# Yash-10/beta-sgp

Measured on AMD Instinct MI355X. Metric: SGP iterations/sec (fp64) on batched 256x256 images, higher is better.
Workload: dtype f64; 1 GPU; C3: 1024 independent 256x256 stamps per GPU, 25x25 PSF, linear A, beta-SGP (beta=1.05), proj_type=1, MAXIT=100, stop_criterion=1; images_per_gpu=1024, images_total=1024, maxit=100, parallelism=1 independent shards, one process per GPU (no collective on the data path), ls_spec=2, streams=1, team=1, proj_cache=1, gn_compact=1, storage=f64, persistent=1, stop_criterion=1

## Files before the change

beta-sgp_amd/csrc/bsgp_device.hpp:

```cpp
#pragma once

#include <hip/hip_runtime.h>
#include <stdint.h>

#include <type_traits>

#include "bsgp_fft.hpp"
#include "bsgp_math.hpp"

namespace bsgp {

#ifndef BSGP_BLOCK
#define BSGP_BLOCK 256
#endif
constexpr int kBlock = BSGP_BLOCK;
constexpr int kWaves = kBlock / 64;
constexpr int kMaxRed = 24;

constexpr int kTeamFlags = 64;
constexpr int kPartBufs = 3;
constexpr unsigned long long kPartEmpty = 0xFFF75EE0FFF75EE0ull;
constexpr unsigned int kPartEmptyWord = 0xFFF75EE0u;
constexpr int kSharedBytes = 512;

constexpr int kPhaseSlots = 32;
#ifdef BSGP_PHASE_PROF
static __device__ unsigned long long g_phase[kPhaseSlots];
#define PH_T(v) const unsigned long long v = __builtin_amdgcn_s_memtime()
#define PH_ADD(slot, t0)                                                                 \
  do {                                                                                   \
    if (threadIdx.x == 0) atomicAdd(&g_phase[slot], __builtin_amdgcn_s_memtime() - (t0)); \
  } while (0)
#define PH_SUB(slot, t)                                                                 \
  do {                                                                                  \
    if (PHS >= 0) {                                                                     \
      const unsigned long long t_ = __builtin_amdgcn_s_memtime();                        \
      if (threadIdx.x == 0) atomicAdd(&g_phase[(slot) < 0 ? 0 : (slot)], t_ - (t));       \
      t = t_;                                                                           \
    }                                                                                   \
  } while (0)
#define PH_SUB_T(v) unsigned long long v = __builtin_amdgcn_s_memtime()
#else
#define PH_T(v)
#define PH_ADD(slot, t0)
#define PH_SUB(slot, t)
#define PH_SUB_T(v)
#endif

struct Geo {
  int H, W;
  int P, Q;
  int Qh;
  int nfw;
  int nfc;
  int coop;
  int lpad;
  int sld;
  int tw2;
  int twmix;
  FftPlan fp;
  FftPlan fq;
  const cd* tfA;
  const cd* tfAT;
  size_t tf_stride;
};

__device__ __forceinline__ const cd* tf_of(const Geo& G, int img, int transpose) {
  return (transpose ? G.tfAT : G.tfA) + (size_t)img * G.tf_stride;
}

__device__ __forceinline__ void copy_tw(const FftPlan& f) {
  if (f.lds_tw < 0) return;
  extern __shared__ __attribute__((aligned(16))) char bsgp_dyn_lds[];
  cd* d = reinterpret_cast<cd*>(bsgp_dyn_lds + f.lds_tw);
  for (int i = threadIdx.x; i < f.n; i += kBlock) d[i] = f.tw[i];
}
__device__ __forceinline__ void copy_tw2(const FftPlan& f) {
  if (f.lds_tw2 < 0) return;
  extern __shared__ __attribute__((aligned(16))) char bsgp_dyn_lds[];
  cd* d = reinterpret_cast<cd*>(bsgp_dyn_lds + f.lds_tw2);
  const int m = 64 + f.n / 64;
  for (int i = threadIdx.x; i < m; i += blockDim.x) d[i] = f.tw[i < 64 ? i : 64 * (i - 64)];
}
__device__ __forceinline__ void load_tw_lds(const Geo& G) {
  if (G.twmix >= 0) {
    extern __shared__ __attribute__((aligned(16))) char bsgp_dyn_lds[];
    cd* d = reinterpret_cast<cd*>(bsgp_dyn_lds + G.twmix);
    for (int i = threadIdx.x; i < 64 + 512; i += blockDim.x)
      d[i] = G.fp.tw[i < 64 ? 32 * i : 4 * (i - 64)];
  }
// ... 558 lines not shown
    if (v != v) v = __longlong_as_double(0x7ff8000000000000ll);
    st_sc1(slot + (size_t)t.m * kMaxRed, v);
  }
  team_red_barrier(t);
  if (threadIdx.x < 64) {
    const int lane = threadIdx.x;
    double s;
    unsigned int spins = 0;
    for (;;) {
      bool ok = true;
      s = MAX ? -INFINITY : INFINITY;
      for (int mm = lane; mm < t.T; mm += 64) {
        const double u = ld_sc1(slot + (size_t)mm * kMaxRed);
        ok &= !part_empty(u);
        s = MAX ? ((u > s || u != u) ? u : s) : ((u < s || u != u) ? u : s);
      }
      if (red_poll_done(t, ok, spins)) break;
    }
    s = MAX ? wave_max(s) : wave_min(s);
    if (lane == 0) red[kWaves * kMaxRed] = s;
  }
  __syncthreads();
  const double r = red[kWaves * kMaxRed];
  __syncthreads();
  team_red_done(t);
  return r;
}
__device__ __forceinline__ double team_max(double v, double* red, Team& t) {
  return team_ext<true>(v, red, t);
}
__device__ __forceinline__ double team_min(double v, double* red, Team& t) {
  return team_ext<false>(v, red, t);
}

__device__ __forceinline__ double fpow(double x, double a) {
#ifdef BSGP_VALU_X2
  const double x2 = x + 0.0 * a * x;
  const double r1 = exp(a * fast_log(x));
  const double r2 = exp(a * fast_log(x2));
  return r1 == r2 ? r1 : r2;
#else
  return exp(a * fast_log(x));
#endif
}

__device__ __forceinline__ double np_max2(double a, double b) {
  return (a != a || b != b) ? (a + b) : (a > b ? a : b);
}
__device__ __forceinline__ double np_min2(double a, double b) {
  return (a != a || b != b) ? (a + b) : (a < b ? a : b);
}
__device__ __forceinline__ double py_max2(double a, double b) { return (b > a) ? b : a; }
__device__ __forceinline__ double py_min2(double a, double b) { return (b < a) ? b : a; }

struct alignas(32) CPair {
  cd a, b;
};

__device__ __forceinline__ void store_pair(cd* col, bool two, bool pair_ok, cd ak, cd bk) {
  if (two && pair_ok) {
    CPair v;
    v.a = ak;
    v.b = bk;
    *reinterpret_cast<CPair*>(col) = v;
  } else {
    col[0] = ak;
    if (two) col[1] = bk;
  }
}

constexpr int kJCH = 4;
constexpr int kGCH = 3;
constexpr int kPCH = 5;

template <int JCH, class LD, class V>
__device__ __forceinline__ void load_rows(LD& ld, int r, bool two, int j0, int lane, int ncols,
                                          V (&v0)[JCH], V (&v1)[JCH]) {
  const int r1 = two ? r + 1 : r;
#pragma unroll
  for (int u = 0; u < JCH; ++u) {
    const int j = min(j0 + lane + 64 * u, ncols - 1);
    v0[u] = ld(r, j);
    v1[u] = ld(r1, j);
  }
}

struct BlockSync {
  __device__ __forceinline__ void operator()() const { __syncthreads(); }
};
constexpr int kCCH = 4;


template <class LD, class MK>
__device__ __forceinline__ void coop_row_fwd_1(const Geo& G, const Part& D, int nrows, int ncols,
                                             int ldim, cd* spec, cd* lds, LD& ld, MK& mk) {
  using V = decltype(ld(0, 0));
  const int t = threadIdx.x;
  const bool pair_ok = (ldim & 1) == 0;
  cd* a = lds;
  cd* b = lds + G.lpad;
  for (int r = 2 * D.gw0; r < nrows; r += 2 * D.gws) {
    const bool two = (r + 1) < nrows;
    for (int j0 = 0; j0 < G.Q; j0 += kBlock * kCCH) {
      V v0[kCCH], v1[kCCH];
#pragma unroll
      for (int u = 0; u < kCCH; ++u) {
        const int j = min(j0 + t + kBlock * u, ncols - 1);
        v0[u] = ld(r, j);
        v1[u] = ld(two ? r + 1 : r, j);
      }
#pragma unroll
      for (int u = 0; u < kCCH; ++u) {
        const int j = j0 + t + kBlock * u;
        if (j < G.Q) {
          double va = 0.0, vb = 0.0;
          if (j < ncols) {
            va = mk(r, j, v0[u]);
            if (two) vb = mk(r + 1, j, v1[u]);
          }
          a[j] = cmk(va, vb);
        }
      }
    }
    __syncthreads();
    cd* Z = fft_wide(a, b, G.fq, false, t, kBlock, BlockSync());
    for (int k = t; k < G.Qh; k += kBlock) {
      cd ak, bk;
      r2c_split(Z, G.Q, k, &ak, &bk);
      store_pair(spec + (size_t)k * ldim + r, two, pair_ok, ak, bk);
    }
    __syncthreads();
  }
}

__device__ __forceinline__ void coop_gather_1(const Geo& G, const cd* spec, int r, bool two, cd* a) {
  const int t = threadIdx.x;
  for (int k0 = 0; k0 < G.Qh; k0 += kBlock * kCCH) {
    cd A[kCCH], B[kCCH];
#pragma unroll
    for (int u = 0; u < kCCH; ++u) {
      const int k = min(k0 + t + kBlock * u, G.Qh - 1);
      const cd* col = spec + (size_t)k * G.sld + r;
      A[u] = col[0];
      const cd b = col[two ? 1 : 0];
      B[u] = two ? b : cmk(0.0, 0.0);
    }
#pragma unroll
    for (int u = 0; u < kCCH; ++u) {
      const int k = k0 + t + kBlock * u;
      if (k < G.Qh) {
        a[k] = cmk(A[u].x - B[u].y, A[u].y + B[u].x);
        if (k > 0 && G.Q - k >= G.Qh) a[G.Q - k] = cmk(A[u].x + B[u].y, B[u].x - A[u].y);
      }
    }
  }
  __syncthreads();
}

template <class LD, class USE>
__device__ __forceinline__ void coop_row_inv_1(const Geo& G, const Part& D, const cd* spec, cd* lds,
                                             LD& ld, USE& use) {
  using V = decltype(ld(0, 0));
  const int t = threadIdx.x;
  cd* a = lds;
  cd* b = lds + G.lpad;
  for (int r = 2 * D.gw0; r < G.H; r += 2 * D.gws) {
// ... 331 lines not shown
  const int t = c.t;
  cd* a = lds + c.g * 2 * G.lpad;
  cd* b = a + G.lpad;
  for (int k0 = D.gw0; k0 < G.Qh; k0 += D.gws) {
    const int k = k0 + c.g;
    const bool act = k < G.Qh;
    cd* col = spec + (size_t)k * G.sld;
    const cd* tk = tf + (size_t)k * G.P;
    PH_T(tq0);
    if (act) {
      for (int p0 = 0; p0 < G.P; p0 += c.nt * kCCH) {
        cd cv[kCCH];
#pragma unroll
        for (int u = 0; u < kCCH; ++u) {
          const int p = p0 + t + c.nt * u;
          const cd v = col[min(p, G.H - 1)];
          cv[u] = (p < G.H) ? v : cmk(0.0, 0.0);
        }
#pragma unroll
        for (int u = 0; u < kCCH; ++u) {
          const int p = p0 + t + c.nt * u;
          if (p < G.P) a[p] = cv[u];
        }
      }
    }
    __syncthreads();
    PH_ADD(29, tq0);
    PH_T(tq1);
    cd* Z = fft_wide<false>(a, b, G.fp, false, t, c.nt, BlockSync());
    if (act) {
      for (int p0 = 0; p0 < G.P; p0 += c.nt * kCCH) {
        cd tv[kCCH];
#pragma unroll
        for (int u = 0; u < kCCH; ++u) tv[u] = tk[min(p0 + t + c.nt * u, G.P - 1)];
#pragma unroll
        for (int u = 0; u < kCCH; ++u) {
          const int p = p0 + t + c.nt * u;
          if (p < G.P) Z[p] = cmul(Z[p], tv[u]);
        }
      }
    }
    __syncthreads();
    cd* Y = fft_wide<false>(Z, (Z == a) ? b : a, G.fp, true, t, c.nt, BlockSync());
    if (act)
      for (int p = t; p < G.H; p += c.nt) col[p] = Y[p];
    __syncthreads();
    PH_ADD(30, tq1);
  }
}

template <class LD, class MK>
__device__ __forceinline__ void coop_row_fwd(const Geo& G, const Part& D, int nrows, int ncols,
                                             int ldim, cd* spec, cd* lds, LD& ld, MK& mk) {
  if (D.nf == 1)
    coop_row_fwd_1(G, D, nrows, ncols, ldim, spec, lds, ld, mk);
  else
    coop_row_fwd_g(G, D, nrows, ncols, ldim, spec, lds, ld, mk);
}
template <class LD, class USE>
__device__ __forceinline__ void coop_row_inv(const Geo& G, const Part& D, const cd* spec, cd* lds,
                                             LD& ld, USE& use) {
  if (D.nf == 1)
    coop_row_inv_1(G, D, spec, lds, ld, use);
  else
    coop_row_inv_g(G, D, spec, lds, ld, use);
}
template <class CP>
__device__ __forceinline__ void coop_row_inv_fwd(const Geo& G, const Part& D, cd* spec, cd* lds,
                                                 CP& cp) {
  if (D.nf == 1)
    coop_row_inv_fwd_1(G, D, spec, lds, cp);
  else
    coop_row_inv_fwd_g(G, D, spec, lds, cp);
}
__device__ __forceinline__ void coop_col_conv(const Geo& G, const Part& D, cd* spec, const cd* tf,
                                              cd* lds) {
  if (D.nf == 1)
    coop_col_conv_1(G, D, spec, tf, lds);
  else
    coop_col_conv_g(G, D, spec, tf, lds);
}

template <int JCH = kJCH, bool PF = false, bool COMP = true, bool COOP = false,
          bool PIPE = false, int PHS = -1, class LD, class MK>
__device__ __forceinline__ void row_fwd2(const Geo& G, const Part& D, int nrows, int ncols,
                                         int ldim, cd* spec, cd* lds, LD&& ld, MK&& mk) {
  if constexpr (COOP) {
    coop_row_fwd(G, D, nrows, ncols, ldim, spec, lds, ld, mk);
    return;
  }
  using V = decltype(ld(0, 0));
  const int w = threadIdx.x >> 6, lane = threadIdx.x & 63;
  const bool pair_ok = (ldim & 1) == 0;
  if (w < G.nfw) {
    cd* a = lds + w * 2 * G.lpad;
    cd* b = a + G.lpad;
    int r = 2 * (D.gw0 + w);
    V v0[JCH], v1[JCH];
    if (PF && r < nrows) load_rows<JCH>(ld, r, (r + 1) < nrows, 0, lane, ncols, v0, v1);
    PH_SUB_T(tph);
    for (; r < nrows; r += 2 * D.gws) {
      const bool two = (r + 1) < nrows;
      auto put = [&](int j0, const V (&w0)[JCH], const V (&w1)[JCH]) __attribute__((always_inline)) {
#pragma unroll
        for (int u = 0; u < JCH; ++u) {
          const int j = j0 + lane + 64 * u;
          if (j < G.Q) {
            double va = 0.0, vb = 0.0;
            if (j < ncols) {
              va = mk(r, j, w0[u]);
              if (two) vb = mk(r + 1, j, w1[u]);
            }
            a[j] = cmk(va, vb);
          }
        }
      };
      if constexpr (PIPE) {
        constexpr int S = 64 * JCH;
        V u0[JCH], u1[JCH];
        if (!PF) load_rows<JCH>(ld, r, two, 0, lane, ncols, v0, v1);
        for (int j0 = 0; j0 < G.Q; j0 += 2 * S) {
          if (j0 + S < ncols) load_rows<JCH>(ld, r, two, j0 + S, lane, ncols, u0, u1);
          put(j0, v0, v1);
          if (j0 + S < G.Q) {
            if (j0 + 2 * S < ncols) load_rows<JCH>(ld, r, two, j0 + 2 * S, lane, ncols, v0, v1);
            put(j0 + S, u0, u1);
          }
        }
      } else {
        for (int j0 = 0; j0 < G.Q; j0 += 64 * JCH) {
          if ((!PF || j0 > 0) && j0 < ncols) load_rows<JCH>(ld, r, two, j0, lane, ncols, v0, v1);
          put(j0, v0, v1);
        }
      }
      const int rn = r + 2 * D.gws;
      if (PF && rn < nrows) load_rows<JCH>(ld, rn, (rn + 1) < nrows, 0, lane, ncols, v0, v1);
      wave_sync();
      PH_SUB(PHS, tph);
      cd* Z = fft_any<COMP>(a, b, G.fq, false, lane, 64, WaveSync());
      PH_SUB(PHS + 1, tph);
      for (int k = lane; k < G.Qh; k += 64) {
        cd ak, bk;
        r2c_split(Z, G.Q, k, &ak, &bk);
        store_pair(spec + (size_t)k * ldim + r, two, pair_ok, ak, bk);
      }
      wave_sync();
      PH_SUB(PHS + 2, tph);
    }
  }
}

template <bool COOP = false, class Prod>
__device__ __forceinline__ void row_fwd(const Geo& G, const Part& D, int nrows, int ncols, int ldim,
                                        cd* spec, cd* lds, Prod&& prod) {
  row_fwd2<kJCH, false, true, COOP>(G, D, nrows, ncols, ldim, spec, lds, prod,
                                                  [](int, int, double v) { return v; });
}

__device__ __forceinline__ void gather_pair(const Geo& G, const cd* spec, int ld, int r, bool two,
                                            cd* a, int lane) {
  for (int k0 = lane; k0 < G.Qh; k0 += 64 * kGCH) {
    cd A[kGCH], B[kGCH];
#pragma unroll
    for (int u = 0; u < kGCH; ++u) {
      const int k = min(k0 + 64 * u, G.Qh - 1);
      const cd* col = spec + (size_t)k * ld + r;
      A[u] = col[0];
      const cd bk = col[two ? 1 : 0];
      B[u] = two ? bk : cmk(0.0, 0.0);
    }
#pragma unroll
    for (int u = 0; u < kGCH; ++u) {
      const int k = k0 + 64 * u;
      if (k < G.Qh) {
        a[k] = cmk(A[u].x - B[u].y, A[u].y + B[u].x);
        if (k > 0 && G.Q - k >= G.Qh) a[G.Q - k] = cmk(A[u].x + B[u].y, B[u].x - A[u].y);
      }
    }
  }
}

typedef __attribute__((address_space(3))) void lds_void_t;
typedef __attribute__((address_space(1))) void gbl_void_t;
__device__ __forceinline__ void stage_pair(const Geo& G, const cd* spec, int ld, int r, bool two,
                                           cd* F, int lane) {
  for (int k0 = 0; k0 < G.Qh; k0 += 64) {
    const int k = k0 + lane;
    if (k < G.Qh) {
      const cd* col = spec + (size_t)k * ld + r;
      __builtin_amdgcn_global_load_lds((gbl_void_t*)col, (lds_void_t*)(F + k0), 16, 0, 0);
      if (two)
        __builtin_amdgcn_global_load_lds((gbl_void_t*)(col + 1), (lds_void_t*)(F + G.Qh + k0), 16,
                                         0, 0);
    }
  }
}
__device__ __forceinline__ void unpack_pair(const Geo& G, const cd* F, bool two, cd* a, int lane) {
  for (int k = lane; k < G.Qh; k += 64) {
    const cd A = F[k];
    const cd B = two ? F[G.Qh + k] : cmk(0.0, 0.0);
    a[k] = cmk(A.x - B.y, A.y + B.x);
    if (k > 0 && G.Q - k >= G.Qh) a[G.Q - k] = cmk(A.x + B.y, B.x - A.y);
  }
}

template <bool PRE, int JCH = kJCH, bool COMP = true, bool COOP = false,
          bool PIPE = false, int PHS = -1, class LD, class USE>
__device__ __forceinline__ void row_inv2(const Geo& G, const Part& D, const cd* spec, cd* lds,
                                         LD&& ld, USE&& use) {
  if constexpr (COOP) {
    coop_row_inv(G, D, spec, lds, ld, use);
    return;
  }
  using V = decltype(ld(0, 0));
  const int w = threadIdx.x >> 6, lane = threadIdx.x & 63;
  if (w < G.nfw) {
    cd* in = lds + w * 2 * G.lpad;
    cd* other = in + G.lpad;
    int r = 2 * (D.gw0 + w);
    PH_SUB_T(tph);
    if (r < G.H) gather_pair(G, spec, G.sld, r, (r + 1) < G.H, in, lane);
    for (; r < G.H; r += 2 * D.gws) {
      const bool two = (r + 1) < G.H;
      V v0[JCH], v1[JCH];
      if (PRE) load_rows<JCH>(ld, r, two, 0, lane, G.W, v0, v1);
      wave_sync();
      PH_SUB(PHS + 2, tph);
      cd* Z = fft_any<COMP>(in, other, G.fq, true, lane, 64, WaveSync());
      PH_SUB(PHS + 1, tph);
      cd* F = (Z == in) ? other : in;
      const int rn = r + 2 * D.gws;
      const bool next = rn < G.H, two_n = (rn + 1) < G.H;
      if (next) stage_pair(G, spec, G.sld, rn, two_n, F, lane);
      auto eat = [&](int j0, const V (&w0)[JCH], const V (&w1)[JCH]) __attribute__((always_inline)) {
#pragma unroll
        for (int u = 0; u < JCH; ++u) {
          const int j = j0 + lane + 64 * u;
          if (j < G.W) {
            const cd z = Z[j];
            use(r, j, z.x, w0[u]);
            if (two) use(r + 1, j, z.y, w1[u]);
          }
        }
      };
      if constexpr (PIPE) {
        constexpr int S = 64 * JCH;
        V u0[JCH], u1[JCH];
        if (!PRE) load_rows<JCH>(ld, r, two, 0, lane, G.W, v0, v1);
        for (int j0 = 0; j0 < G.W; j0 += 2 * S) {
          load_rows<JCH>(ld, r, two, j0 + S, lane, G.W, u0, u1);
          eat(j0, v0, v1);
          if (j0 + S < G.W) {
            load_rows<JCH>(ld, r, two, j0 + 2 * S, lane, G.W, v0, v1);
            eat(j0 + S, u0, u1);
          }
        }
      } else {
        for (int j0 = 0; j0 < G.W; j0 += 64 * JCH) {
          if (!PRE || j0 > 0) load_rows<JCH>(ld, r, two, j0, lane, G.W, v0, v1);
          eat(j0, v0, v1);
        }
      }
      PH_SUB(PHS, tph);
      if (next) {
        asm volatile("s_waitcnt vmcnt(0)" ::: "memory");
        wave_sync();
        unpack_pair(G, F, two_n, Z, lane);
        in = Z;
        other = F;
      }
    }
    wave_sync();
  }
}

template <bool COOP = false, class Cons>
__device__ __forceinline__ void row_inv(const Geo& G, const Part& D, const cd* spec, cd* lds,
                                        Cons&& cons) {
  row_inv2<false, kJCH, true, COOP>(
      G, D, spec, lds, [](int, int) { return 0; },
      [&](int r, int j, double v, int) { cons(r, j, v); });
}

template <bool COOP = false, class CP>
__device__ __forceinline__ void row_inv_fwd(const Geo& G, const Part& D, cd* spec, cd* lds,
                                            CP&& cp) {
  if constexpr (COOP) {
    coop_row_inv_fwd(G, D, spec, lds, cp);
    return;
  }
  const int w = threadIdx.x >> 6, lane = threadIdx.x & 63;
  const bool pair_ok = (G.sld & 1) == 0;
  if (w < G.nfw) {
    cd* a = lds + w * 2 * G.lpad;
    cd* b = a + G.lpad;
    for (int r = 2 * (D.gw0 + w); r < G.H; r += 2 * D.gws) {
      const bool two = (r + 1) < G.H;
      gather_pair(G, spec, G.sld, r, two, a, lane);
      wave_sync();
      cd* Z = fft_any(a, b, G.fq, true, lane, 64, WaveSync());
      cd* in2 = (Z == a) ? b : a;
      for (int j = lane; j < G.Q; j += 64) {
        double va = 0.0, vb = 0.0;
        if (j < G.W) {
          const cd z = Z[j];
          va = cp(r, j, z.x);
          if (two) vb = cp(r + 1, j, z.y);
        }
        in2[j] = cmk(va, vb);
      }
      wave_sync();
      cd* Y = fft_any(in2, Z, G.fq, false, lane, 64, WaveSync());
      for (int k = lane; k < G.Qh; k += 64) {
        cd ak, bk;
        r2c_split(Y, G.Q, k, &ak, &bk);
        store_pair(spec + (size_t)k * G.sld + r, two, pair_ok, ak, bk);
      }
      wave_sync();
    }
  }
}

template <bool COOP = false>
__device__ __forceinline__ void col_conv(const Geo& G, const Part& D, cd* spec, const cd* tf,
                                         cd* lds) {
  if constexpr (COOP) {
    coop_col_conv(G, D, spec, tf, lds);
    return;
  }
  const int w = threadIdx.x >> 6, lane = threadIdx.x & 63;
  if (w < G.nfw) {
    cd* a = lds + w * 2 * G.lpad;
    cd* b = a + G.lpad;
    for (int k = D.gw0 + w; k < G.Qh; k += D.gws) {
      cd* col = spec + (size_t)k * G.sld;
      const cd* t = tf + (size_t)k * G.P;
      for (int p0 = 0; p0 < G.P; p0 += 64 * kPCH) {
        cd cv[kPCH];
#pragma unroll
        for (int u = 0; u < kPCH; ++u) {
          const int p = p0 + lane + 64 * u;
          const cd c = col[min(p, G.H - 1)];
          cv[u] = p < G.H ? c : cmk(0.0, 0.0);
        }
#pragma unroll
        for (int u = 0; u < kPCH; ++u) {
          const int p = p0 + lane + 64 * u;
          if (p < G.P) a[p] = cv[u];
        }
      }
      wave_sync();
      cd* Z = fft_any(a, b, G.fp, false, lane, 64, WaveSync());
      if (G.P <= 64 * kPCH) {
        cd tv[kPCH];
#pragma unroll
// ... 324 lines not shown
```

beta-sgp_amd/csrc/bsgp_kernels.hpp:

```cpp
#pragma once

#include <hip/hip_runtime.h>

#include <type_traits>
#include <vector>

#include "bsgp_device.hpp"
#include "bsgp_internal.hpp"

namespace bsgp {


#ifndef BSGP_LS1_PRE
#define BSGP_LS1_PRE false
#endif
constexpr int kLs1Jch = 1;
#ifndef BSGP_COL_ATTR
#define BSGP_COL_ATTR
#endif
#ifndef BSGP_LS_ATTR
#define BSGP_LS_ATTR __attribute__((amdgpu_waves_per_eu(COOP ? 1 : ((K <= 2 && !ADAPT) ? 3 : 2))))
#endif
#ifndef BSGP_LS1_K2
#define BSGP_LS1_K2 0
#endif
constexpr int kLsLanes = 32;
#ifndef BSGP_ACC_SERIES
#define BSGP_ACC_SERIES 0
#endif
constexpr int kLsAccJch = 1;
constexpr bool kLsAccPf = true;
#ifndef BSGP_LS1_PIPE
#define BSGP_LS1_PIPE false
#endif
#ifndef BSGP_LSACC_PIPE
#define BSGP_LSACC_PIPE false
#endif
#ifndef BSGP_BB_PIPE
#define BSGP_BB_PIPE false
#endif
constexpr int kProjU = 4;
constexpr int kDirJch = 4;
constexpr bool kDirPf = true;
constexpr bool kDirComp = true;
constexpr bool kLsComp = false;
constexpr bool kBbComp = false;
#ifndef BSGP_BB_PRE
#define BSGP_BB_PRE false
#endif
constexpr int kBbJch = 1;

__device__ __forceinline__ double clipX(double x, double lo, double hi) {
  double X = (x < lo) ? lo : x;
  return (X > hi) ? hi : X;
}

__device__ __forceinline__ double realtime_s() {
  return (double)__builtin_amdgcn_s_memrealtime() * 1e-8;
}

template <int U, class LD, class CP>
__device__ __forceinline__ void stream_range(int p0, int p1, LD&& ld, CP&& cp) {
  using T = decltype(ld(0));
  for (int b = p0 + threadIdx.x; b < p1; b += kBlock * U) {
    T v[U];
#pragma unroll
    for (int u = 0; u < U; ++u) v[u] = ld(min(b + u * kBlock, p1 - 1));
#pragma unroll
    for (int u = 0; u < U; ++u) {
      const int p = b + u * kBlock;
      if (p < p1) cp(p, v[u]);
    }
  }
}
template <int U, class LD, class CP>
__device__ __forceinline__ void stream2(const Part& D, int npair, LD&& ld, CP&& cp) {
  if (D.T == 1) {
    stream_range<U>(0, npair, ld, cp);
    return;
  }
  for (int p0 = D.m * D.cp; p0 < npair; p0 += D.T * D.cp)
    stream_range<U>(p0, p0 + D.cp < npair ? p0 + D.cp : npair, ld, cp);
}

__device__ __forceinline__ double2 ld2(const double* a, int p) {
  return reinterpret_cast<const double2*>(a)[p];
}
__device__ __forceinline__ double2 ld2(const float* a, int p) {
  const float2 f = reinterpret_cast<const float2*>(a)[p];
  return double2{(double)f.x, (double)f.y};
}

template <class T>
__device__ __forceinline__ double opt_ld(bool on, const T* a, int i, double off) {
  const double v = (double)a[on ? i : 0];
  return on ? v : off;
}
__device__ __forceinline__ double2 opt_ld2(bool on, const double* a, int p, double off) {
  const double2 v = ld2(a, on ? p : 0);
  return on ? v : double2{off, off};
}
__device__ __forceinline__ double g_raw(bool g32, const double* gns, int i) {
  const unsigned int* w = reinterpret_cast<const unsigned int*>(gns) + (g32 ? i : 2 * i);
  unsigned long long u;
  __builtin_memcpy(&u, __builtin_assume_aligned(w, 4), 8);
  return __longlong_as_double((long long)u);
}
__device__ __forceinline__ double2 g_raw2(bool g32, const double* gns, int p) {
  const double* a = g32 ? gns + p : gns + 2 * p;
  double2 v;
  __builtin_memcpy(&v, __builtin_assume_aligned(a, 8), 16);
  return v;
}

template <class V>
struct Bufs {
  double *gns, *bks;
  V *xa, *xb, *ga, *gb, *xtf, *dtf;
  V* pw;
  cd* spec;
};

template <class V>
__device__ __forceinline__ Bufs<V> slot_bufs(const SolveArgs& A, int img, int par) {
  Bufs<V> b;
  double* ws = A.ws + (size_t)img * A.slot_stride;
  const size_t v = A.vec_stride;
  b.gns = ws;
  b.bks = ws + v;
  V* vb = reinterpret_cast<V*>(ws + 2 * v);
  V* x0 = vb;
  V* x1 = vb + v;
  V* g0 = vb + 2 * v;
  V* g1 = vb + 3 * v;
  b.xa = par ? x1 : x0;
  b.xb = par ? x0 : x1;
  b.ga = par ? g1 : g0;
  b.gb = par ? g0 : g1;
  b.xtf = vb + 4 * v;
  b.dtf = vb + 5 * v;
  b.pw = vb + 6 * v;
  b.spec = reinterpret_cast<cd*>(ws + A.spec_off);
  return b;
}

struct Dir {
  bool Xones, proj;
  double alpha, lo, hi, lam_p;
  ProjClip clip;
  __device__ __forceinline__ void cd_of(double x, double g, double& c, double& dia) const {
    const double X = Xones ? 1.0 : clipX(x, lo, hi);
    const double D = 1 / X;
    const double y = x - alpha * (X * g);
    c = y * D;
    dia = D;
  }
  __device__ __forceinline__ void yx(double x, double g, double& y, double& X) const {
    X = Xones ? 1.0 : clipX(x, lo, hi);
    y = x - alpha * (X * g);
  }
  __device__ __forceinline__ double pv(double y, double X, double lam) const {
    double v = fma(lam, X, y);
    v = (0.0 > v) ? 0.0 : v;
    if (clip.has_sat) v = (clip.satv < v) ? clip.satv : v;
    return v;
  }
  __device__ __forceinline__ double d(double x, double g) const {
    double y;
    if (proj) {
      double c, dia;
      cd_of(x, g, c, dia);
      y = clip(c, dia, lam_p);
    } else {
      const double X = Xones ? 1.0 : clipX(x, lo, hi);
      y = x - alpha * (X * g);
      if (y < 0) y = 0;
    }
    return y - x;
  }
};

// ... 546 lines not shown
        (void)pass(std::integral_constant<int, 1>{}, lams, Sv, split, qL, qU);
        S = Sv[0];
      }
    }
    ++calls;
    note(lam, S);
    return S;
  };
  return project_df_fn(sumf, flux, 0.0, 1.0, 1e-11, 0, 0, A.prm.max_projs);
}

template <bool COOP, class V, bool LL = true>
__device__ __forceinline__ void dir_phase(const SolveArgs& A, int img) {
  BSGP_LDS_VIEWS(A);
  ImgState& st = A.st[img];
  PH_T(tk0);
  Team tm = make_team(A, img, st);
  const Geo& G = A.g;
  const Part Pt = make_part(tm, G.nfw, G.W);
  const bsgp_params& P = A.prm;
  const int N = G.H * G.W;
  const int npair = (N + 1) / 2;
  const bool odd = (N & 1) != 0;
  Bufs<V> B = slot_bufs<V>(A, img, st.par);
  Dir D = make_dir(A, st);
  const double flux = st.flux;
  int evals = 0;
  int64_t ppass = 0, plist_reads = 0;
  double lam_ratio = 0.0, kappa = 0.0;
  if (P.proj_type == 1 && A.plist != nullptr) {
    double first_lam = NAN;
    ProjOut po = cached_projection<V, LL>(A, img, Pt, tm, D, B, red, lds, st.lam_p, flux, npair,
                                          odd, N, ppass, plist_reads, st.lam_ratio, st.kappa,
                                          first_lam);
    D.lam_p = po.lam;
    evals = po.evals;
    lam_ratio = D.alpha != 0.0 ? po.lam / D.alpha : 0.0;
    kappa = (isfinite(first_lam) && po.lam != 0.0) ? first_lam / po.lam : 0.0;
  } else if (P.proj_type == 1) {
    const V* xa = B.xa;
    const V* ga = B.ga;
    auto psum = [&](double lam) {
      double s[1] = {0.0};
      stream2<4>(
          Pt, npair,
          [&](int p) {
            struct Ld {
              double2 x, g;
            } v;
            v.x = ld2(xa, p);
            v.g = ld2(ga, p);
            return v;
          },
          [&](int p, const auto& v) {
            double c, d;
            D.cd_of(v.x.x, v.g.x, c, d);
            s[0] += D.clip(c, d, lam);
            if (!odd || 2 * p + 1 < N) {
              D.cd_of(v.x.y, v.g.y, c, d);
              s[0] += D.clip(c, d, lam);
            }
          });
      team_sum<1>(s, red, tm);
      return s[0];
    };
    ProjOut po = project_df_fn(psum, flux, 0.0, 1.0, 1e-11, 0, 0, P.max_projs);
    D.lam_p = po.lam;
    evals = po.evals;
    ppass = po.evals;
  }
  PH_ADD(0, tk0);
  PH_T(tk1);
  double gd[1] = {0.0};
  row_fwd2<kDirJch, kDirPf, kDirComp, COOP, false, 22>(
      G, Pt, G.H, G.W, G.sld, B.spec, lds,
      [&](int r, int j) {
        const int i = r * G.W + j;
        return double2{B.xa[i], B.ga[i]};
      },
      [&](int, int, const double2& v) {
        const double d = D.d(v.x, v.y);
        gd[0] += d * v.y;
        return d;
      });
  team_sum<1>(gd, red, tm);
  PH_ADD(1, tk1);
  PH_ADD(2, tk0);
  team_end(st, tm);
  if (leader(tm)) {
    for (int k = 0; k < P.M_alpha - 1; ++k) st.Valpha[k] = st.Valpha[k + 1];
    for (int k = 0; k < P.M - 1; ++k) st.Fold[k] = st.Fold[k + 1];
    st.Fold[P.M - 1] = st.fv;
    st.epoch += 1;
    st.lam_p = D.lam_p;
    st.lam_ratio = isfinite(lam_ratio) ? lam_ratio : 0.0;
    st.kappa = isfinite(kappa) ? kappa : 0.0;
    st.E_p += evals;
    st.proj_passes += ppass;
    st.proj_list += plist_reads;
    st.gd = gd[0];
  }
}

template <bool COOP, class V>
__global__ void __launch_bounds__(kBlock) k_dir(SolveArgs A) {
  const int img = team_img(A);
  if (A.st[img].stop) return;
  load_tw_lds(A.g);
  dir_phase<COOP, V>(A, img);
}

template <bool COOP>
__global__ void __launch_bounds__(kBlock) BSGP_COL_ATTR k_col(SolveArgs A, int transpose) {
  BSGP_LDS_VIEWS(A);
  const int img = A.img0 + (A.Tc == 1 ? (int)blockIdx.x : (int)(blockIdx.x / (unsigned)A.Tc));
  const ImgState& st = A.st[img];
  if (st.stop) return;
  PH_T(tc0);
  Team tm{};
  tm.T = A.Tc;
  tm.m = A.Tc == 1 ? 0 : (int)(blockIdx.x % (unsigned)A.Tc);
  const Bufs<double> B = slot_bufs<double>(A, img, 0);
  load_tw_lds(A.g);
  col_conv<COOP>(A.g, make_part(tm, A.g.nfc, A.g.W), B.spec, tf_of(A.g, img, transpose), lds);
  PH_ADD(3, tc0);
}

template <int K, int MODE, bool ADAPT, bool COOP, class V, bool SB = false>
__device__ __forceinline__ void ls_phase(const SolveArgs& A, int img) {
  BSGP_LDS_VIEWS(A);
  ImgState& st = A.st[img];
  PH_T(tk0);
  Team tm = make_team(A, img, st);
  const Geo& G = A.g;
  const Part Pt = make_part(tm, G.nfw, G.W);
  const bsgp_params& P = A.prm;
  const int N = G.H * G.W;
  const int npair = (N + 1) / 2;
  const bool odd = (N & 1) != 0;
  const bool bmap = SB ? false : P.bkg_is_map != 0;
  const double lr_st = st.lr;
  constexpr bool adapt = ADAPT;
  Bufs<V> B = slot_bufs<V>(A, img, st.par);
  const double bks_scalar = st.bks_scalar;
  const double flux = st.flux;
  const double gd = st.gd;
  const int g32 = st.g32;
  const double gsc = st.sc, grc = 1.0 / st.sc, gfill = st.gfill;
  auto gdec1 = [&](float v) __attribute__((always_inline)) {
    const double g = v;
    return g > 0 ? (g32 == 2 ? div_rn(g, gsc, grc) : g) : gfill;
  };
  auto gdec = [&](double r) __attribute__((always_inline)) {
    return g32 ? gdec1(__int_as_float(__double2loint(r))) : r;
  };
  double fr = st.Fold[0];
  for (int k = 1; k < P.M; ++k) fr = py_max2(fr, st.Fold[k]);
  const int ls_cap = A.ls_cap;
  Objective obj = make_obj(A, st.beta);
  double lam = 1.0;
  double f_acc = 0.0;
  int nls = 0, passes = 0, status = 0, series_evals = 0;
  bool accepted = false;
  bool acc_series = false;
  constexpr int NT = 2 * K + 2;
  double konst = st.konst;
  const bool k32 = ADAPT && P.gn_f32 != 0;
// ... 328 lines not shown
  team_end(st, tm);
  if (leader(tm)) {
    if (A.out.flags)
      A.out.flags[(size_t)img * (P.MAXIT + 1) + st.iter] =
          ((f_acc >= fr) ? 1 : 0) | ((nls < 0xffff ? nls : 0xffff) << 8);
    st.fv = f_acc;
    st.beta = obj.beta;
    st.konst = konst;
    st.lam = lam_acc;
    st.E_ls += nls;
    st.ls_passes += passes;
    st.ls_series += series_evals;
    st.status |= status;
  }
}

template <int K, int MODE, bool ADAPT, bool COOP, class V>
__global__ void __launch_bounds__(kBlock) BSGP_LS_ATTR k_ls(SolveArgs A) {
  const int img = team_img(A);
  if (A.st[img].stop) return;
  load_tw_lds(A.g);
  ls_phase<K, MODE, ADAPT, COOP, V>(A, img);
}


template <bool COOP, class V>
__device__ __forceinline__ void bb_phase(const SolveArgs& A, int img) {
  BSGP_LDS_VIEWS(A);
  ImgState& st = A.st[img];
  PH_T(tk0);
  Team tm = make_team(A, img, st);
  const Geo& G = A.g;
  const Part Pt = make_part(tm, G.nfw, G.W);
  const bsgp_params& P = A.prm;
  const int N = G.H * G.W;
  const int tid = threadIdx.x;
  const bool beta_obj = P.variant == BSGP_VARIANT_BETA;
  Bufs<V> B = slot_bufs<V>(A, img, st.par);
  Dir D = make_dir(A, st);
  const double lam = st.lam;
  const double lo = st.lo, hi = st.hi;
  const double alpha = st.alpha;
  double vmin_ring = INFINITY;
  for (int k = 0; k < P.M_alpha - 1; ++k) vmin_ring = k ? py_min2(vmin_ring, st.Valpha[k]) : st.Valpha[0];
  const int iter = st.iter;
  const double tau0 = st.tau, init_lr = st.init_lr, lr0 = st.lr;
  const int epoch = st.epoch;
  const double fv = st.fv, Dcoeff = st.Dcoeff, tol = st.tol, fold_last = st.Fold[P.M - 1];
  const double sc = st.sc;
  double bb[6] = {0, 0, 0, 0, 0, 0};
  struct BbIn {
    double p, x, g;
  };
  row_inv2<BSGP_BB_PRE, kBbJch, kBbComp, COOP, BSGP_BB_PIPE, 19>(
      G, Pt, B.spec, lds,
      [&](int r, int j) {
        const int i = r * G.W + j;
        BbIn q;
        q.p = opt_ld(beta_obj, B.pw, i, 1.0);
        q.x = B.xa[i];
        q.g = B.ga[i];
        return q;
      },
      [&](int r, int j, double at, const BbIn& q) {
    const int i = r * G.W + j;
    const double gnew = q.p - at;
    const double x = q.x, g = q.g;
    const double d = D.d(x, g);
    const double sk = lam * d;
    const double xn = x + lam * d;
    const double yk = gnew - g;
    const double X = clipX(xn, lo, hi);
    const double Dd = 1 / X;
    const double sk2 = sk * Dd;
    const double yk2 = yk * X;
    bb[0] += sk2 * yk;
    bb[1] += yk2 * sk;
    bb[2] += sk2 * sk2;
    bb[3] += yk2 * yk2;
    bb[4] += sk * sk;
    bb[5] += xn * xn;
    B.xb[i] = xn;
    B.gb[i] = gnew;
  });
  team_sum<6>(bb, red, tm);
  PH_ADD(8, tk0);
  double alpha1, alpha2;
  if (bb[0] <= 0) {
    alpha1 = py_min2(10 * alpha, P.alpha_max);
  } else {
    alpha1 = py_min2(P.alpha_max, py_max2(P.alpha_min, bb[2] / bb[0]));
  }
  if (bb[1] <= 0) {
    alpha2 = py_min2(10 * alpha, P.alpha_max);
  } else {
    alpha2 = py_min2(P.alpha_max, py_max2(P.alpha_min, bb[1] / bb[3]));
  }
  const double vmin = P.M_alpha > 1 ? py_min2(vmin_ring, alpha2) : alpha2;
  double tau = tau0, anew;
  if (iter <= 20) {
    anew = vmin;
  } else if (alpha2 / alpha1 < tau) {
    anew = vmin;
    tau = tau * 0.9;
  } else {
    anew = alpha1;
    tau = tau * 1.1;
  }
  const double lr = (P.variant == BSGP_VARIANT_BETA && P.schedule_lr)
                        ? init_lr * exp(-P.lr_exp_param * epoch)
                        : lr0;
  const int it2 = iter + 1;
  bool loop = true;
  double crit = 0.0;
  const double dk = Dcoeff * fv;
  if (P.stop_criterion == 2) {
    crit = bb[4] / bb[5];
    loop = crit > tol;
  } else if (P.stop_criterion == 3) {
    crit = (fold_last - fv) / fv;
    loop = crit > tol && crit >= 0;
  } else if (P.stop_criterion == 4) {
    crit = dk;
    loop = dk > tol;
  }
  if (it2 > P.MAXIT) loop = false;
  if (!loop) {
    double* xo = A.out.x + (size_t)img * N;
    for (int i = Pt.gt0 + tid; i < N; i += Pt.gts) xo[i] = B.xa[i] * sc;
  }
  team_end(st, tm);
  if (leader(tm)) {
    const size_t M1 = (size_t)P.MAXIT + 1;
    A.out.discr[img * M1 + it2 - 1] = dk;
    if (A.out.times) A.out.times[img * M1 + it2 - 1] = realtime_s() - st.t0;
    if (A.out.crit) A.out.crit[img * M1 + it2 - 1] = crit;
    st.Valpha[P.M_alpha - 1] = alpha2;
    st.alpha = anew;
    st.tau = tau;
    st.lr = lr;
    st.iter = it2;
    if (loop) {
      st.par ^= 1;
      st.Xones = 0;
    } else {
      st.stop = 1;
      A.out.iters[img] = it2 - 1;
      if (A.out.beta_final) A.out.beta_final[img] = st.beta;
      write_counters(A, st, img, tm.T);
      count_stopped(A);
    }
  }
}

template <bool COOP, class V>
__global__ void __launch_bounds__(kBlock) k_bb(SolveArgs A) {
  const int img = team_img(A);
  if (A.st[img].stop) return;
  load_tw_lds(A.g);
  bb_phase<COOP, V>(A, img);
}

static __global__ void k_ring_init(unsigned* queue, int nimg, int img0) {
  unsigned long long* ring = reinterpret_cast<unsigned long long*>(queue + 4);
  const int i = blockIdx.x * blockDim.x + threadIdx.x;
  if (i == 0) {
    queue[0] = 0;
// ... 375 lines not shown
```

Baseline: 278,400 image-iterations/s.

## Widen row loads to paired 16-byte loads with permlane32 lane split

Row-pass FFT loaders in the direction and BB-sum stages now read two adjacent columns per lane as 16-byte vector loads. The lower half-wave loads row r and the upper half loads row r+1, and permlane32_swap then redistributes the values so each lane holds both rows for its column. Lane-to-column mapping changes, so per-lane reduction partials are shuffled back before the team sums. Separately, stage_pair interleaves the two spectrum rows in LDS with one async global-to-LDS load per lane instead of two predicated loads. The aim is fewer, wider global transactions, paid for with extra swap and shuffle instructions and a second template instantiation.

```diff
diff --git a/beta-sgp_amd/csrc/bsgp_device.hpp b/beta-sgp_amd/csrc/bsgp_device.hpp
--- a/beta-sgp_amd/csrc/bsgp_device.hpp
+++ b/beta-sgp_amd/csrc/bsgp_device.hpp
@@ -6,6 +6,7 @@
 #include <type_traits>
 
 #include "bsgp_fft.hpp"
+#include "bsgp_lanesplit.hpp"
 #include "bsgp_math.hpp"
 
 namespace bsgp {
@@ -730,6 +731,50 @@
     const int j = min(j0 + lane + 64 * u, ncols - 1);
     v0[u] = ld(r, j);
     v1[u] = ld(r1, j);
+  }
+}
+
+template <class V>
+struct Two {
+  V a, b;
+};
+struct NoWide {};
+
+template <class T>
+__device__ __forceinline__ void half_swap(T& a, T& b) {
+  static_assert(sizeof(T) % 4 == 0, "whole dwords");
+  constexpr int N = sizeof(T) / 4;
+  unsigned int x[N], y[N];
+  __builtin_memcpy(x, &a, sizeof(T));
+  __builtin_memcpy(y, &b, sizeof(T));
+#pragma unroll
+  for (int n = 0; n < N; ++n) {
+    const auto s = __builtin_amdgcn_permlane32_swap(x[n], y[n], false, false);
+    x[n] = s[0];
+    y[n] = s[1];
+  }
+  __builtin_memcpy(&a, x, sizeof(T));
+  __builtin_memcpy(&b, y, sizeof(T));
+}
+
+template <bool COOP>
+__device__ __forceinline__ bool row_wide(const Geo& G) {
+  return !COOP && (G.W & 1) == 0;
+}
+
+__device__ __forceinline__ double split_undo(double v) {
+  return __shfl(v, split_lane((int)(threadIdx.x & 63u)), 64);
+}
+
+template <int JCH, class LD2, class V>
+__device__ __forceinline__ void load_rows2(LD2& ld2, int r, bool two, int j0, int lane, int ncols,
+                                           V (&v0)[JCH], V (&v1)[JCH]) {
+  const int rr = (two && split_half(lane)) ? r + 1 : r;
+#pragma unroll
+  for (int u = 0; u < JCH; ++u) {
+    const Two<V> q = ld2(rr, split_pair_clamped(j0 + 64 * u, lane, ncols));
+    v0[u] = q.a;
+    v1[u] = q.b;
   }
 }
 
@@ -1227,9 +1272,10 @@
 }
 
 template <int JCH = kJCH, bool PF = false, bool COMP = true, bool COOP = false,
-          bool PIPE = false, int PHS = -1, class LD, class MK>
+          bool PIPE = false, int PHS = -1, class LD, class MK, class LD2 = NoWide>
 __device__ __forceinline__ void row_fwd2(const Geo& G, const Part& D, int nrows, int ncols,
-                                         int ldim, cd* spec, cd* lds, LD&& ld, MK&& mk) {
+                                         int ldim, cd* spec, cd* lds, LD&& ld, MK&& mk,
+                                         LD2&& ld2 = LD2{}) {
   if constexpr (COOP) {
     coop_row_fwd(G, D, nrows, ncols, ldim, spec, lds, ld, mk);
     return;
@@ -1237,24 +1283,36 @@
   using V = decltype(ld(0, 0));
   const int w = threadIdx.x >> 6, lane = threadIdx.x & 63;
   const bool pair_ok = (ldim & 1) == 0;
+  constexpr bool kHasWide =
+      !std::is_same<typename std::decay<LD2>::type, NoWide>::value;
   if (w < G.nfw) {
+    auto run = [&](auto wide_c, auto& ldw) __attribute__((always_inline)) {
+    constexpr bool WIDE = decltype(wide_c)::value;
+    auto load = [&](int rr, bool two_r, int j0, V (&w0)[JCH], V (&w1)[JCH]) __attribute__((always_inline)) {
+      if constexpr (WIDE)
+        load_rows2<JCH>(ldw, rr, two_r, j0, lane, ncols, w0, w1);
+      else
+        load_rows<JCH>(ld, rr, two_r, j0, lane, ncols, w0, w1);
+    };
     cd* a = lds + w * 2 * G.lpad;
     cd* b = a + G.lpad;
     int r = 2 * (D.gw0 + w);
     V v0[JCH], v1[JCH];
-    if (PF && r < nrows) load_rows<JCH>(ld, r, (r + 1) < nrows, 0, lane, ncols, v0, v1);
+    if (PF && r < nrows) load(r, (r + 1) < nrows, 0, v0, v1);
     PH_SUB_T(tph);
     for (; r < nrows; r += 2 * D.gws) {
       const bool two = (r + 1) < nrows;
       auto put = [&](int j0, const V (&w0)[JCH], const V (&w1)[JCH]) __attribute__((always_inline)) {
 #pragma unroll
         for (int u = 0; u < JCH; ++u) {
-          const int j = j0 + lane + 64 * u;
+          V q0 = w0[u], q1 = w1[u];
+          if constexpr (WIDE) half_swap(q0, q1);
+          const int j = j0 + 64 * u + (WIDE ? split_col(lane) : lane);
           if (j < G.Q) {
             double va = 0.0, vb = 0.0;
             if (j < ncols) {
-              va = mk(r, j, w0[u]);
-              if (two) vb = mk(r + 1, j, w1[u]);
+              va = mk(r, j, q0);
+              if (two) vb = mk(r + 1, j, q1);
             }
             a[j] = cmk(va, vb);
           }
@@ -1263,23 +1321,23 @@
       if constexpr (PIPE) {
         constexpr int S = 64 * JCH;
         V u0[JCH], u1[JCH];
-        if (!PF) load_rows<JCH>(ld, r, two, 0, lane, ncols, v0, v1);
+        if (!PF) load(r, two, 0, v0, v1);
         for (int j0 = 0; j0 < G.Q; j0 += 2 * S) {
-          if (j0 + S < ncols) load_rows<JCH>(ld, r, two, j0 + S, lane, ncols, u0, u1);
+          if (j0 + S < ncols) load(r, two, j0 + S, u0, u1);
           put(j0, v0, v1);
           if (j0 + S < G.Q) {
-            if (j0 + 2 * S < ncols) load_rows<JCH>(ld, r, two, j0 + 2 * S, lane, ncols, v0, v1);
+            if (j0 + 2 * S < ncols) load(r, two, j0 + 2 * S, v0, v1);
             put(j0 + S, u0, u1);
           }
         }
       } else {
         for (int j0 = 0; j0 < G.Q; j0 += 64 * JCH) {
-          if ((!PF || j0 > 0) && j0 < ncols) load_rows<JCH>(ld, r, two, j0, lane, ncols, v0, v1);
+          if ((!PF || j0 > 0) && j0 < ncols) load(r, two, j0, v0, v1);
           put(j0, v0, v1);
         }
       }
       const int rn = r + 2 * D.gws;
-      if (PF && rn < nrows) load_rows<JCH>(ld, rn, (rn + 1) < nrows, 0, lane, ncols, v0, v1);
+      if (PF && rn < nrows) load(rn, (rn + 1) < nrows, 0, v0, v1);
       wave_sync();
       PH_SUB(PHS, tph);
       cd* Z = fft_any<COMP>(a, b, G.fq, false, lane, 64, WaveSync());
@@ -1292,6 +1350,15 @@
       wave_sync();
       PH_SUB(PHS + 2, tph);
     }
+    };
+    if constexpr (kHasWide) {
+      if ((ncols & 1) == 0)
+        run(std::true_type{}, ld2);
+      else
+        run(std::false_type{}, ld2);
+    } else {
+      run(std::false_type{}, ld2);
+    }
   }
 }
 
@@ -1329,37 +1396,44 @@
 typedef __attribute__((address_space(1))) void gbl_void_t;
 __device__ __forceinline__ void stage_pair(const Geo& G, const cd* spec, int ld, int r, bool two,
                                            cd* F, int lane) {
-  for (int k0 = 0; k0 < G.Qh; k0 += 64) {
-    const int k = k0 + lane;
+  for (int k0 = 0; k0 < G.Qh; k0 += 32) {
+    const int k = k0 + (lane >> 1);
     if (k < G.Qh) {
-      const cd* col = spec + (size_t)k * ld + r;
-      __builtin_amdgcn_global_load_lds((gbl_void_t*)col, (lds_void_t*)(F + k0), 16, 0, 0);
-      if (two)
-        __builtin_amdgcn_global_load_lds((gbl_void_t*)(col + 1), (lds_void_t*)(F + G.Qh + k0), 16,
-                                         0, 0);
+      const cd* col = spec + (size_t)k * ld + r + (two ? (lane & 1) : 0);
+      __builtin_amdgcn_global_load_lds((gbl_void_t*)col, (lds_void_t*)(F + 2 * k0), 16, 0, 0);
     }
   }
 }
 __device__ __forceinline__ void unpack_pair(const Geo& G, const cd* F, bool two, cd* a, int lane) {
   for (int k = lane; k < G.Qh; k += 64) {
-    const cd A = F[k];
-    const cd B = two ? F[G.Qh + k] : cmk(0.0, 0.0);
+    const cd A = F[2 * k];
+    const cd B = two ? F[2 * k + 1] : cmk(0.0, 0.0);
     a[k] = cmk(A.x - B.y, A.y + B.x);
     if (k > 0 && G.Q - k >= G.Qh) a[G.Q - k] = cmk(A.x + B.y, B.x - A.y);
   }
 }
 
 template <bool PRE, int JCH = kJCH, bool COMP = true, bool COOP = false,
-          bool PIPE = false, int PHS = -1, class LD, class USE>
+          bool PIPE = false, int PHS = -1, class LD, class USE, class LD2 = NoWide>
 __device__ __forceinline__ void row_inv2(const Geo& G, const Part& D, const cd* spec, cd* lds,
-                                         LD&& ld, USE&& use) {
+                                         LD&& ld, USE&& use, LD2&& ld2 = LD2{}) {
   if constexpr (COOP) {
     coop_row_inv(G, D, spec, lds, ld, use);
     return;
   }
   using V = decltype(ld(0, 0));
   const int w = threadIdx.x >> 6, lane = threadIdx.x & 63;
+  constexpr bool kHasWide =
+      !std::is_same<typename std::decay<LD2>::type, NoWide>::value;
   if (w < G.nfw) {
+    auto run = [&](auto wide_c, auto& ldw) __attribute__((always_inline)) {
+    constexpr bool WIDE = decltype(wide_c)::value;
+    auto load = [&](int rr, bool two_r, int j0, V (&w0)[JCH], V (&w1)[JCH]) __attribute__((always_inline)) {
+      if constexpr (WIDE)
+        load_rows2<JCH>(ldw, rr, two_r, j0, lane, G.W, w0, w1);
+      else
+        load_rows<JCH>(ld, rr, two_r, j0, lane, G.W, w0, w1);
+    };
     cd* in = lds + w * 2 * G.lpad;
     cd* other = in + G.lpad;
     int r = 2 * (D.gw0 + w);
@@ -1368,7 +1442,7 @@
     for (; r < G.H; r += 2 * D.gws) {
       const bool two = (r + 1) < G.H;
       V v0[JCH], v1[JCH];
-      if (PRE) load_rows<JCH>(ld, r, two, 0, lane, G.W, v0, v1);
+      if (PRE) load(r, two, 0, v0, v1);
       wave_sync();
       PH_SUB(PHS + 2, tph);
       cd* Z = fft_any<COMP>(in, other, G.fq, true, lane, 64, WaveSync());
@@ -1380,29 +1454,31 @@
       auto eat = [&](int j0, const V (&w0)[JCH], const V (&w1)[JCH]) __attribute__((always_inline)) {
 #pragma unroll
         for (int u = 0; u < JCH; ++u) {
-          const int j = j0 + lane + 64 * u;
+          V q0 = w0[u], q1 = w1[u];
+          if constexpr (WIDE) half_swap(q0, q1);
+          const int j = j0 + 64 * u + (WIDE ? split_col(lane) : lane);
           if (j < G.W) {
             const cd z = Z[j];
-            use(r, j, z.x, w0[u]);
-            if (two) use(r + 1, j, z.y, w1[u]);
+            use(r, j, z.x, q0);
+            if (two) use(r + 1, j, z.y, q1);
           }
         }
       };
       if constexpr (PIPE) {
         constexpr int S = 64 * JCH;
         V u0[JCH], u1[JCH];
-        if (!PRE) load_rows<JCH>(ld, r, two, 0, lane, G.W, v0, v1);
+        if (!PRE) load(r, two, 0, v0, v1);
         for (int j0 = 0; j0 < G.W; j0 += 2 * S) {
-          load_rows<JCH>(ld, r, two, j0 + S, lane, G.W, u0, u1);
+          load(r, two, j0 + S, u0, u1);
           eat(j0, v0, v1);
           if (j0 + S < G.W) {
-            load_rows<JCH>(ld, r, two, j0 + 2 * S, lane, G.W, v0, v1);
+            load(r, two, j0 + 2 * S, v0, v1);
             eat(j0 + S, u0, u1);
           }
         }
       } else {
         for (int j0 = 0; j0 < G.W; j0 += 64 * JCH) {
-          if (!PRE || j0 > 0) load_rows<JCH>(ld, r, two, j0, lane, G.W, v0, v1);
+          if (!PRE || j0 > 0) load(r, two, j0, v0, v1);
           eat(j0, v0, v1);
         }
       }
@@ -1416,6 +1492,15 @@
       }
     }
     wave_sync();
+    };
+    if constexpr (kHasWide) {
+      if ((G.W & 1) == 0)
+        run(std::true_type{}, ld2);
+      else
+        run(std::false_type{}, ld2);
+    } else {
+      run(std::false_type{}, ld2);
+    }
   }
 }
 
diff --git a/beta-sgp_amd/csrc/bsgp_kernels.hpp b/beta-sgp_amd/csrc/bsgp_kernels.hpp
--- a/beta-sgp_amd/csrc/bsgp_kernels.hpp
+++ b/beta-sgp_amd/csrc/bsgp_kernels.hpp
@@ -96,7 +96,8 @@
   const double v = (double)a[on ? i : 0];
   return on ? v : off;
 }
-__device__ __forceinline__ double2 opt_ld2(bool on, const double* a, int p, double off) {
+template <class T>
+__device__ __forceinline__ double2 opt_ld2(bool on, const T* a, int p, double off) {
   const double2 v = ld2(a, on ? p : 0);
   return on ? v : double2{off, off};
 }
@@ -809,7 +810,13 @@
         const double d = D.d(v.x, v.y);
         gd[0] += d * v.y;
         return d;
+      },
+      [&](int r, int j) {
+        const int p = (r * G.W + j) >> 1;
+        const double2 x = ld2(B.xa, p), g = ld2(B.ga, p);
+        return Two<double2>{double2{x.x, g.x}, double2{x.y, g.y}};
       });
+  if (row_wide<COOP>(G)) gd[0] = split_undo(gd[0]);
   team_sum<1>(gd, red, tm);
   PH_ADD(1, tk1);
   PH_ADD(2, tk0);
@@ -1304,7 +1311,16 @@
     bb[5] += xn * xn;
     B.xb[i] = xn;
     B.gb[i] = gnew;
-  });
+  },
+      [&](int r, int j) {
+        const int p = (r * G.W + j) >> 1;
+        const double2 pw = opt_ld2(beta_obj, B.pw, p, 1.0), x = ld2(B.xa, p), g = ld2(B.ga, p);
+        return Two<BbIn>{BbIn{pw.x, x.x, g.x}, BbIn{pw.y, x.y, g.y}};
+      });
+  if (row_wide<COOP>(G)) {
+#pragma unroll
+    for (int k = 0; k < 6; ++k) bb[k] = split_undo(bb[k]);
+  }
   team_sum<6>(bb, red, tm);
   PH_ADD(8, tk0);
   double alpha1, alpha2;
diff --git a/beta-sgp_amd/csrc/bsgp_lanesplit.hpp b/beta-sgp_amd/csrc/bsgp_lanesplit.hpp
--- /dev/null
+++ b/beta-sgp_amd/csrc/bsgp_lanesplit.hpp
@@ -0,0 +1,19 @@
+#pragma once
+
+#if defined(__HIPCC__) || defined(__CUDACC__)
+#define BSGP_SPLIT_HD __host__ __device__
+#else
+#define BSGP_SPLIT_HD
+#endif
+
+namespace bsgp {
+
+BSGP_SPLIT_HD constexpr int split_half(int lane) { return lane >> 5; }
+BSGP_SPLIT_HD constexpr int split_pair(int lane) { return 2 * (lane & 31); }
+BSGP_SPLIT_HD constexpr int split_pair_clamped(int j0, int lane, int ncols) {
+  return (j0 + split_pair(lane) < ncols - 2) ? j0 + split_pair(lane) : ncols - 2;
+}
+BSGP_SPLIT_HD constexpr int split_col(int lane) { return 2 * (lane & 31) + (lane >> 5); }
+BSGP_SPLIT_HD constexpr int split_lane(int L) { return (L >> 1) | ((L & 1) << 5); }
+
+}
```

Measured after the change: 281,300 image-iterations/s (median of 6 runs). +1.0%, better.
